# eRGiBi/DRL-DroneNavigation

Measured on AMD Instinct MI355X. Metric: env_steps_per_sec, higher is better.
Workload: dtype f64

## Files before the change

drl-dronenavigation_amd/csrc/dn_kernels.hip:

```cpp
#include "dn_internal.h"
#include "dn_action_sat.h"

#ifndef DN_TU
#define DN_TU 1
#endif

#include <float.h>
#include <type_traits>

#define DN_DEV __device__ __forceinline__

namespace {

template <typename R> struct K {
    static constexpr R M = R(0.027);
    static constexpr R IXX = R(1.4e-5), IYY = R(1.4e-5), IZZ = R(2.17e-5);
    static constexpr R G = R(9.8);
    static constexpr R DT = R(1.0 / 240.0);
    static constexpr R ARM = R(0.028);
    static constexpr R LIN_DAMP = R(0.04), ANG_DAMP = R(0.04);
    static constexpr R MAX_COORD_VEL = R(100.0);
    static constexpr R PI = R(3.14159265358979323846);
    static constexpr R COLL_R = R(0.06), COLL_H = R(0.025);
    static constexpr R INV_M = R(1.0 / 0.027);
// ... 543 lines not shown
    s = FM<R>::fma(s, h2, R(-1.0 / 6.0));
    sinc = FM<R>::fma(s, h2, R(1.0));
    R k = R(1.0 / 479001600.0);
    k = FM<R>::fma(k, h2, R(-1.0 / 3628800.0));
    k = FM<R>::fma(k, h2, R(1.0 / 40320.0));
    k = FM<R>::fma(k, h2, R(-1.0 / 720.0));
    k = FM<R>::fma(k, h2, R(1.0 / 24.0));
    k = FM<R>::fma(k, h2, R(-0.5));
    c = FM<R>::fma(k, h2, R(1.0));
}

struct Meta {
    int steps, idx, just_found;
};
DN_DEV Meta unpack_meta(float f)
{
    unsigned u = __float_as_uint(f);
    Meta m;
    m.steps = (int)(u & 0xFFFFFFu);
    m.idx = (int)((u >> 24) & 0x7Fu);
    m.just_found = (int)(u >> 31);
    return m;
}
DN_DEV float pack_meta(int steps, int idx, int just_found)
{
    return __uint_as_float(((unsigned)steps & 0xFFFFFFu) | (((unsigned)idx & 0x7Fu) << 24) | ((unsigned)just_found << 31));
}

struct StepOut {
    float *obs;
    float *reward;
    uint8_t *done, *truncated;
    int32_t *found;
    float *terminal_obs;
    float *ep_return;
    int32_t *ep_length;
    unsigned long long *done_word;
};
DN_DEV StepOut block_out(const DnStepIO &io, long long tile_base, long long step_off, long long word_off)
{
    StepOut o;
    const long long e = step_off + tile_base;
    o.obs = io.obs + e * DN_OBS_DIM;
    o.reward = io.reward + e;
    o.done = io.done + e;
    o.truncated = io.truncated + e;
    o.found = io.found_targets + e;
    o.terminal_obs = io.terminal_obs ? io.terminal_obs + e * DN_OBS_DIM : nullptr;
    o.ep_return = io.ep_return ? io.ep_return + e : nullptr;
    o.ep_length = io.ep_length ? io.ep_length + e : nullptr;
    o.done_word = io.done_mask ? io.done_mask + word_off + tile_base / DN_BLOCK : nullptr;
    return o;
}

DN_DEV void pin(double &x) { asm volatile("" : "+v"(x)); }
DN_DEV void pin(float &x) { asm volatile("" : "+v"(x)); }
DN_DEV void pin(bool &x) { int t = x; asm volatile("" : "+v"(t)); x = t != 0; }

DN_DEV void wave_lds_sync()
{
    __builtin_amdgcn_fence(__ATOMIC_RELEASE, "wavefront");
    __builtin_amdgcn_s_waitcnt(0xc07f);
    __builtin_amdgcn_wave_barrier();
    __builtin_amdgcn_fence(__ATOMIC_ACQUIRE, "wavefront");
}
DN_DEV void block_lds_barrier()
{
    __builtin_amdgcn_fence(__ATOMIC_RELEASE, "workgroup", "local");
    __builtin_amdgcn_s_barrier();
    __builtin_amdgcn_fence(__ATOMIC_ACQUIRE, "workgroup", "local");
}

DN_DEV void tile_park(float *s_tile, unsigned lane, const float o[DN_OBS_DIM])
{
    asm volatile("" ::: "memory");
#pragma unroll
    for (int k = 0; k < DN_OBS_DIM; ++k) s_tile[lane * DN_OBS_DIM + k] = o[k];
    asm volatile("" ::: "memory");
}
struct TileRegs {
    float4 r[4];
};
DN_DEV TileRegs tile_fetch(const float *s_tile, unsigned lane)
{
    asm volatile("" ::: "memory");
    const float4 *s4 = reinterpret_cast<const float4 *>(s_tile);
    TileRegs t;
#pragma unroll
    for (int r = 0; r < 3; ++r) t.r[r] = s4[r * 64 + lane];
    t.r[3] = s4[192 + (lane < (DN_BLOCK * DN_OBS_DIM / 4 - 192) ? lane : 0)];
    asm volatile("" ::: "memory");
    return t;
}
DN_DEV void tile_stream(const TileRegs &t, const float *s_tile, float *gtile, unsigned rows, unsigned lane)
{
    if (rows == DN_BLOCK) {
        float4 *g4 = reinterpret_cast<float4 *>(gtile);
#pragma unroll
        for (int r = 0; r < 3; ++r) g4[r * 64 + lane] = t.r[r];
        if (lane < (DN_BLOCK * DN_OBS_DIM / 4 - 192)) g4[192 + lane] = t.r[3];
    } else {
        const unsigned rem = rows * DN_OBS_DIM;
        for (unsigned e = lane; e < rem; e += DN_BLOCK) gtile[e] = s_tile[e];
    }
}
DN_DEV void store_obs_tile(float *s_tile, float *gtile, unsigned rows, unsigned lane, const float o[DN_OBS_DIM])
{
    tile_park(s_tile, lane, o);
    const TileRegs t = tile_fetch(s_tile, lane);
// ... 1176 lines not shown
        const double inv = rcp_f64(tot);
        const double delta = rn.returns - rn.mean;
        rn.mean = __builtin_fma(delta, inv, rn.mean);
        rn.var = __builtin_fma(delta * delta, inv, rn.var) * (rn.count * inv);
        rn.count = tot;
        const double s = rn.var + 1e-8;
        double y = __builtin_amdgcn_rsq(s);
        y = __builtin_fma(y, __builtin_fma(-(0.5 * s * y), y, 0.5), y);
        y = __builtin_fma(y, __builtin_fma(-(0.5 * s * y), y, 0.5), y);
        r = r * y;
        if (done) rn.returns = 0.0;
    }
    return r;
}

DN_DEV long long fixed6(double x)
{
    const double m = x * 1e6 + 6755399441055744.0;
    return __double_as_longlong(m) - 0x4338000000000000ll;
}

struct StatAcc {
    long long episodes = 0, truncated = 0, completed = 0, sum_len = 0, sum_found = 0, sum_ret_fix = 0;
};
DN_DEV void flush_stats(const DnParams &p, const StatAcc &a, unsigned long long steps_after, unsigned lane)
{
    if (lane == 0) {
        DnStatSlot sl = p.st.stats[blockIdx.x];
        sl.episodes += a.episodes; sl.truncated += a.truncated; sl.completed += a.completed;
        sl.sum_len += a.sum_len; sl.sum_found += a.sum_found; sl.sum_ret_fix += a.sum_ret_fix;
        sl.step_count = steps_after;
        p.st.stats[blockIdx.x] = sl;
    }
}
DN_DEV void flush_stats_preloaded(const DnParams &p, DnStatSlot sl, const StatAcc &a, unsigned long long steps_after, unsigned lane,
                                  const long long tile)
{
    if (lane == 0) {
        sl.episodes += a.episodes; sl.truncated += a.truncated; sl.completed += a.completed;
        sl.sum_len += a.sum_len; sl.sum_found += a.sum_found; sl.sum_ret_fix += a.sum_ret_fix;
        sl.step_count = steps_after;
        p.st.stats[tile] = sl;
    }
}

struct __attribute__((packed, aligned(4))) ObsQuad { float x, y, z, w; };
DN_DEV void store_obs_direct(float *row, const float o[DN_OBS_DIM])
{
    *reinterpret_cast<ObsQuad *>(row) = ObsQuad{o[0], o[1], o[2], o[3]};
    *reinterpret_cast<ObsQuad *>(row + 4) = ObsQuad{o[4], o[5], o[6], o[7]};
    *reinterpret_cast<ObsQuad *>(row + 8) = ObsQuad{o[8], o[9], o[10], o[11]};
    row[12] = o[12];
}
DN_DEV float ret_lo(const float hi, const int lenword)
{
    const int eb = (__float_as_int(hi) >> 23) & 0xFF;
    return (float)(lenword >> 24) * __int_as_float((eb > 31 ? eb - 31 : 0) << 23);
}
DN_DEV int ret_lo_byte(const double ep_ret, const float hi)
{
    const int eb = (__float_as_int(hi) >> 23) & 0xFF;
    const bool ok = eb > 31 && eb < 255;
    const float inv = __int_as_float((ok ? 285 - eb : 127) << 23);
    const double q = __builtin_rint((ep_ret - (double)hi) * (double)inv);
    const int k = (int)fmin(fmax(q, -128.0), 127.0);
    return ok ? (k & 0xFF) : 0;
}
template <typename R, bool REW, bool FOUND_BIT = false, bool BANK = false>
DN_DEV void report_scalars(const DnParams &p, const DnConsts<R> &c, const StepOut &out, const Flight<R> &fl, const Verdict<R> &v,
                           const R r_normal, const float r_found32, const unsigned li, const unsigned lane, const bool active,
                           float4 &G4, float4 &G5, StatAcc &acc, RewNorm &rn, const bool found_mail = false, const int W_lane = 0,
                           unsigned long long *track_count = nullptr, const int track_e = 0)
{
    const bool coll1 = v.coll1 != 0, terminated = v.terminated != 0, truncated = fl.truncated != 0;
    const bool found_now = !coll1 && (FOUND_BIT ? found_mail : (R)fl.d_e <= c.threshold);
    const bool is_done = found_now && fl.idx_e + 1 == (BANK ? W_lane : p.num_waypoints);
    const int found = fl.idx_e + (found_now ? 1 : 0);
    const bool done = terminated || truncated;
    R reward;
    if (coll1) reward = R(-10.0);
    else if (found_now) reward = (R)(r_found32 / 25.0f);
    else reward = r_normal * K<R>::INV_25;
    if (REW) reward = (R)reward_wrappers(p, rn, (double)reward, done);
    const int lenword = __float_as_int(G5.w);
    const int eplen_e = lenword & 0xFFFFFF;
    R ep_ret = ((R)G4.w + (R)ret_lo(G4.w, lenword)) + reward;
    int ep_len = eplen_e + 1;
    float4 S4 = G4, S5 = G5;
    if (!terminated) {
        S4 = make_float4(fl.vex, fl.vey, fl.vez, 0.0f);
        S5 = make_float4(fl.aex, fl.aey, fl.aez, 0.0f);
    }
    const unsigned long long done_ballot = __ballot(done && active);
    if (done_ballot != 0ull) {
        const long long fix = fixed6((double)ep_ret);
        if (done) {
            if (active) {
                if (out.ep_return) out.ep_return[li] = (float)ep_ret;
                if (out.ep_length) out.ep_length[li] = ep_len;
            }
            S4 = S5 = make_float4(0.0f, 0.0f, 0.0f, 0.0f);
            ep_ret = R(0.0); ep_len = 0;
        }
        const long long n_trunc = __popcll(__ballot(done && active && truncated && !terminated));
        const long long n_compl = __popcll(__ballot(done && active && is_done));
        long long s_len = 0, s_fd = 0, s_ret = 0;
        const int fix_lo = (int)(unsigned)(fix & 0xFFFFFFFFll), fix_hi = (int)(fix >> 32);
        for (unsigned long long m = done_ballot; m != 0ull; m &= m - 1ull) {
            const int l = __builtin_ctzll(m);
            s_len += (long long)__builtin_amdgcn_readlane(eplen_e, l) + 1;
            s_fd += (long long)__builtin_amdgcn_readlane(found, l);
            const unsigned lo = (unsigned)__builtin_amdgcn_readlane(fix_lo, l);
            const int hi = __builtin_amdgcn_readlane(fix_hi, l);
            s_ret += (long long)(((unsigned long long)(unsigned)hi << 32) | lo);
        }
        acc.episodes += __popcll(done_ballot); acc.truncated += n_trunc; acc.completed += n_compl;
        acc.sum_len += s_len; acc.sum_found += s_fd; acc.sum_ret_fix += s_ret;
        if constexpr (BANK) if (track_count) {
            for (unsigned long long left = done_ballot; left != 0ull;) {
                const int t = __builtin_amdgcn_readlane(track_e, __builtin_ctzll(left));
                const bool mine = done && active && track_e == t;
                const unsigned long long same = __ballot(mine);
                const unsigned long long c_compl = __popcll(__ballot(mine && is_done)), c_trunc = __popcll(__ballot(mine && truncated && !terminated));
                unsigned long long t_len = 0, t_fd = 0;
                for (unsigned long long m = same; m != 0ull; m &= m - 1ull) {
                    const int l = __builtin_ctzll(m);
                    t_len += (unsigned long long)(__builtin_amdgcn_readlane(eplen_e, l) + 1);
                    t_fd += (unsigned long long)__builtin_amdgcn_readlane(found, l);
                }
                if (lane == 0) {
                    unsigned long long *cnt = track_count + 5 * t;
                    track_count_add(cnt + 0, (unsigned long long)__popcll(same));
                    if (c_compl) track_count_add(cnt + 1, c_compl);
                    if (c_trunc) track_count_add(cnt + 2, c_trunc);
                    track_count_add(cnt + 3, t_fd);
                    track_count_add(cnt + 4, t_len);
                }
                left &= ~same;
            }
        }
    }
    S4.w = (float)ep_ret; S5.w = __int_as_float(ep_len | (ret_lo_byte((double)ep_ret, S4.w) << 24));
    G4 = S4; G5 = S5;
    if (active) {
        out.reward[li] = (float)reward;
        out.done[li] = (uint8_t)done;
        out.truncated[li] = (uint8_t)(truncated && !terminated);
        out.found[li] = found;
    }
    if (out.done_word && lane == 0) *out.done_word = done_ballot;
}
template <typename R, bool NORM, bool NOISE, int TILE, bool SPAWN = false, int M = DN_M_NONE>
DN_DEV void report_obs(const DnParams &p, const DnConsts<R> &c, float *s_tile, const StepOut &out, const bool truncated,
                       const Verdict<R> &v, float *o, const unsigned long long gid, const unsigned long long step_count,
                       const unsigned li, const unsigned lane, const unsigned rows, const bool active, Rms &rms, SensCtx *sx = nullptr,
                       const PrivCtx *px = nullptr, const GoalCtx<R> *gx = nullptr)
{
    constexpr bool SENS = M >= DN_M_SENS, PRIV = M >= DN_M_PRIV, GOAL = M >= DN_M_GOAL;
    const bool done = v.terminated != 0 || truncated;
    const unsigned long long done_mask = __ballot(done && active);
    if (done_mask != 0ull) {
        const bool across = NOISE && TILE == 2 && s_tile != nullptr && p.obs_noise_sigma > 0.0f;
        float zr[DN_OBS_DIM];
        if (across) draw_obs_noise_across(p, gid - li, step_count, 5u, done_mask, done && active, lane, s_tile, zr);
        if (done) {
            if (active && out.terminal_obs) {
#pragma unroll
                for (int k = 0; k < DN_OBS_DIM; ++k) out.terminal_obs[li * DN_OBS_DIM + k] = o[k];
            }
            reset_obs<R>(p, c, v.d_obs, o);
            if (SPAWN && p.random_spawn) {
                double q[3];
                spawn_point(p, gid, step_count, q);
#pragma unroll
                for (int k = 0; k < 3; ++k) o[k] = (float)((R)(float)q[k] * c.inv_dim[k]);
            }
            if constexpr (PRIV) {
                if ((px->pv->groups & DN_PRIV_OBS) && active) priv_store_obs(px->row, o);
            }
            if (across) add_obs_noise_drawn(p, zr, o);
            else if (NOISE && p.obs_noise_sigma > 0.0f) add_obs_noise(p, gid, step_count, 5u, o);
            if constexpr (SENS) {
                if (sx->sn->lat_on || sx->sn->bias_on)
                    sens_restart(*sx->sn, sx->n, sx->i, sx->active, p.seed, gid, step_count, sens_slot(*sx->sn, step_count), sx->d, o);
            }
            if constexpr (GOAL) {
                if (active && gx->row) goal_store<R>(*gx->g, gx->rW, c, gx->tab + gx->roff, gx->row, o, 0);
            }
            if (NORM) normalize_obs(rms, o);
        }
    }
    if (TILE == 2) { if (active) store_obs_direct(out.obs + li * DN_OBS_DIM, o); }
    else if (TILE == 1) tile_park(s_tile, lane, o);
    else store_obs_tile(s_tile, out.obs, rows, lane, o);
}
template <typename R, bool NORM, bool NOISE, bool REW, int TILE = 0, bool SPAWN = false, int M = DN_M_NONE>
DN_DEV void report_phase(const DnParams &p, const DnConsts<R> &c, float *s_tile, const StepOut &out, const Flight<R> &fl,
                         const Verdict<R> &v, Observed<R> &ob, const unsigned long long gid, const unsigned long long step_count,
                         const unsigned li, const unsigned lane, const unsigned rows, const bool active,
                         float4 &G4, float4 &G5, StatAcc &acc, Rms &rms, RewNorm &rn, SensCtx *sx = nullptr, const PrivCtx *px = nullptr,
                         const GoalCtx<R> *gx = nullptr, unsigned long long *track_count = nullptr, const int track_e = 0)
{
    if constexpr (M >= DN_M_GOAL) report_scalars<R, REW, false, true>(p, c, out, fl, v, ob.r_normal, ob.r_found32, li, lane, active, G4, G5, acc, rn, false, gx->W,
                                                                      track_count, track_e);
    else report_scalars<R, REW>(p, c, out, fl, v, ob.r_normal, ob.r_found32, li, lane, active, G4, G5, acc, rn);
    report_obs<R, NORM, NOISE, TILE, SPAWN, M>(p, c, s_tile, out, fl.truncated != 0, v, ob.o, gid, step_count, li, lane, rows, active,
                                                              rms, sx, px, gx);
}

struct BlockState {
    float4 *g0, *g1, *g2, *g3, *g4, *g5, *g6, *g7;
};
DN_DEV BlockState block_state(const DnState &st, long long tile_base)
{
    BlockState b;
    b.g0 = st.g0 + tile_base; b.g1 = st.g1 + tile_base; b.g2 = st.g2 + tile_base; b.g3 = st.g3 + tile_base;
    b.g4 = st.g4 + tile_base; b.g5 = st.g5 + tile_base; b.g6 = st.g6 + tile_base;
    b.g7 = st.g7 + tile_base;
    return b;
}

// ... 489 lines not shown
            if (XOPT && p.drag) G7 = (v.terminated || fl.truncated) ? make_float4(0.0f, 0.0f, 0.0f, 0.0f) : rpm_now;
            attitude_phase<R>(fl);
            post_mail<R>(mail[t & 1], lane, fl, v);
            block_lds_barrier();
            A = A_next;
        }
        if (active) { b.g0[li] = G0; b.g1[li] = G1; b.g2[li] = G2; b.g3[li] = G3; }
        if (XOPT && p.drag && active) b.g7[li] = G7;
    }
}

template <typename R> struct MailQ {
    R f64[8][DN_BLOCK];
    float4 f32[4][DN_BLOCK];
};
template <typename R> DN_DEV void post_mailq(MailQ<R> &m, unsigned lane, const Flight<R> &f, const Verdict<R> &v)
{
    const R x[8] = {f.px, f.py, f.pz, f.qx, f.qy, f.qz, f.qw, v.d_obs};
#pragma unroll
    for (int k = 0; k < 8; ++k) m.f64[k][lane] = x[k];
    const int fb = f.idx_e | (f.just_found_e << 8) | (f.truncated << 9), vb = v.coll1 | (v.terminated << 1);
    m.f32[0][lane] = make_float4(f.vx, f.vy, f.vz, f.wx);
    m.f32[1][lane] = make_float4(f.wy, f.wz, f.vex, f.vey);
    m.f32[2][lane] = make_float4(f.vez, f.aex, f.aey, f.aez);
    m.f32[3][lane] = make_float4(f.d_e, f.dprev_e, __int_as_float(fb), __int_as_float(vb));
}
template <typename R> DN_DEV void take_mailq(const MailQ<R> &m, unsigned lane, Flight<R> &f, Verdict<R> &v)
{
    R x[8];
#pragma unroll
    for (int k = 0; k < 8; ++k) x[k] = m.f64[k][lane];
    f.px = x[0]; f.py = x[1]; f.pz = x[2]; f.qx = x[3]; f.qy = x[4]; f.qz = x[5]; f.qw = x[6];
    v.d_obs = x[7];
    const float4 a = m.f32[0][lane], b = m.f32[1][lane], c = m.f32[2][lane], d = m.f32[3][lane];
    f.vx = a.x; f.vy = a.y; f.vz = a.z; f.wx = a.w; f.wy = b.x; f.wz = b.y; f.vex = b.z; f.vey = b.w;
    f.vez = c.x; f.aex = c.y; f.aey = c.z; f.aez = c.w; f.d_e = d.x; f.dprev_e = d.y;
    const int bits = __float_as_int(d.z), vb = __float_as_int(d.w);
    f.idx_e = bits & 0xFF; f.just_found_e = (bits >> 8) & 1; f.truncated = (bits >> 9) & 1;
    v.coll1 = vb & 1; v.terminated = (vb >> 1) & 1;
}
template <typename R> struct MailA {
    R f64[2][DN_BLOCK];
    float4 f32[4][DN_BLOCK];
};
template <typename R> DN_DEV void post_maila(MailA<R> &m, unsigned lane, const Flight<R> &f, const Verdict<R> &v, const Observed<R> &ob)
{
    m.f64[0][lane] = ob.r_normal; m.f64[1][lane] = v.d_obs;
    const int bits = f.idx_e | (f.truncated << 9) | (v.coll1 << 10) | (v.terminated << 11);
    m.f32[0][lane] = make_float4(ob.o[0], ob.o[1], ob.o[2], ob.o[3]);
    m.f32[1][lane] = make_float4(ob.o[4], ob.o[5], ob.o[6], ob.o[7]);
    m.f32[2][lane] = make_float4(ob.o[8], ob.o[9], ob.o[10], ob.o[11]);
    m.f32[3][lane] = make_float4(ob.o[12], ob.r_found32, f.d_e, __int_as_float(bits));
}
template <typename R> DN_DEV void take_maila(const MailA<R> &m, unsigned lane, Flight<R> &f, Verdict<R> &v, Observed<R> &ob, int *flag_word = nullptr)
{
    ob.r_normal = m.f64[0][lane]; v.d_obs = m.f64[1][lane];
    const float4 a = m.f32[0][lane], b = m.f32[1][lane], c = m.f32[2][lane], d = m.f32[3][lane];
    ob.o[0] = a.x; ob.o[1] = a.y; ob.o[2] = a.z; ob.o[3] = a.w; ob.o[4] = b.x; ob.o[5] = b.y; ob.o[6] = b.z; ob.o[7] = b.w;
    ob.o[8] = c.x; ob.o[9] = c.y; ob.o[10] = c.z; ob.o[11] = c.w; ob.o[12] = d.x;
    ob.r_found32 = d.y; f.d_e = d.z;
    const int bits = __float_as_int(d.w);
    f.idx_e = bits & 0xFF; f.truncated = (bits >> 9) & 1; v.coll1 = (bits >> 10) & 1; v.terminated = (bits >> 11) & 1;
    f.vex = f.vey = f.vez = f.aex = f.aey = f.aez = 0.0f;
    if (flag_word) *flag_word = bits;
}
constexpr int DN_MAILA_FOUND_SHIFT = 12;
template <typename R> DN_DEV void post_maila_found(MailA<R> &m, unsigned lane, const FlightW<R> &f, const Verdict<R> &v, const Observed<R> &ob,
                                                   const bool found)
{
    m.f64[0][lane] = ob.r_normal; m.f64[1][lane] = v.d_obs;
    const int bits = f.idx_e | (f.truncated << 9) | (v.coll1 << 10) | (v.terminated << 11) | ((int)found << DN_MAILA_FOUND_SHIFT);
    m.f32[0][lane] = make_float4(ob.o[0], ob.o[1], ob.o[2], ob.o[3]);
    m.f32[1][lane] = make_float4(ob.o[4], ob.o[5], ob.o[6], ob.o[7]);
    m.f32[2][lane] = make_float4(ob.o[8], ob.o[9], ob.o[10], ob.o[11]);
    m.f32[3][lane] = make_float4(ob.o[12], ob.r_found32, 0.0f, __int_as_float(bits));
}

template <bool XOPT> struct ThrustMailX { double v[9][DN_BLOCK]; };
template <> struct ThrustMailX<false> { double v[1][1]; };
DN_DEV void post_thrust_x(ThrustMailX<true> &m, unsigned lane, const ThrustX &t, const Extras &x)
{
#pragma unroll
    for (int j = 0; j < 4; ++j) { m.v[j][lane] = t.f[j]; m.v[5 + j][lane] = x.rpm[j]; }
    m.v[4][lane] = t.zt;
}
DN_DEV void take_thrust_x(const ThrustMailX<true> &m, unsigned lane, ThrustX &t, Extras &x)
{
#pragma unroll
    for (int j = 0; j < 4; ++j) { t.f[j] = m.v[j][lane]; x.rpm[j] = m.v[5 + j][lane]; }
    t.zt = m.v[4][lane];
}
DN_DEV void post_thrust_x(ThrustMailX<false> &, unsigned, const ThrustX &, const Extras &) {}
DN_DEV void take_thrust_x(const ThrustMailX<false> &, unsigned, ThrustX &, Extras &) {}
template <typename R, bool XOPT> struct ThrustMailP : ThrustMail<R> {};
template <typename R> struct ThrustMailP<R, true> { R v[1][1]; };
template <typename R> DN_DEV void post_thrust(ThrustMailP<R, true> &, unsigned, const Thrust &) {}
template <typename R> DN_DEV Resultant<R> take_thrust(const ThrustMailP<R, true> &, unsigned) { return Resultant<R>(); }

template <typename R, bool NORM, bool NOISE, bool XOPT>
__global__ __launch_bounds__(3 * DN_BLOCK, NORM ? 2 : 3) void dn_step_many_3w_kernel(const DnParams p, const DnStepIO io0, const int k_steps)
{
    __shared__ ThrustMailX<XOPT> tmx[2];
    __shared__ R s_tab[DN_MAX_WAYPOINTS * DN_T_STRIDE];
    __shared__ __attribute__((aligned(16))) float s_tile[DN_BLOCK * DN_OBS_DIM];
    __shared__ MailQ<R> mailq[2];
    __shared__ MailA<R> maila[2];
    __shared__ __attribute__((aligned(16))) ThrustMailP<R, XOPT> tmail[2];
    const unsigned lane = threadIdx.x & (DN_BLOCK - 1);
    const int wv = __builtin_amdgcn_readfirstlane(threadIdx.x >> 6);
    const int role = wv == 0 ? 0 : (wv == 1 ? 2 : 1);
    const long long tile_base = (long long)blockIdx.x * DN_BLOCK;
    const long long left = p.n - tile_base;
    const unsigned rows = left < DN_BLOCK ? (unsigned)left : DN_BLOCK;
    const bool active = lane < rows;
    const unsigned li = active ? lane : rows - 1;
// ... 120 lines not shown
            reinterpret_cast<float *>(b.g4 + li)[3] = G4.w;
            reinterpret_cast<float *>(b.g5 + li)[3] = G5.w;
            }
    }
}

template <typename R> struct MailL {
    R f64[4][DN_BLOCK];
    R wide[8][DN_BLOCK];
    int flags[DN_BLOCK];
};
template <typename R> struct MailG {
    R col[3][DN_BLOCK];
    R fw[3][DN_BLOCK];
    float4 eul[DN_BLOCK];
    float4 w[DN_BLOCK];
    R we[3][DN_BLOCK];
};

#ifdef DN_MW_STAMP
__device__ long long g_mw_stamp[8][48][2];
#define MW_MARK(k) do { if (lane == 0 && blockIdx.x == DN_MW_STAMP && t >= 8 && t < 56) \
        g_mw_stamp[role][t - 8][k] = (long long)__builtin_readcyclecounter(); } while (0)
#else
#define MW_MARK(k) do { } while (0)
#endif
#define MW_BARRIER() do { MW_MARK(0); block_lds_barrier(); MW_MARK(1); } while (0)
#ifdef DN_ROLE_MARK
#define MW_ROLE_MARK(name) asm volatile("; DN_ROLE_LOOP " name)
#else
#define MW_ROLE_MARK(name) do { } while (0)
#endif
#ifdef DN_MW_STAMP
__device__ long long g_mw_edge[16][8];
#define MW_EDGE(k) do { if (lane == 0 && (blockIdx.x == DN_MW_STAMP || blockIdx.x == DN_MW_STAMP + 256)) { const int r_ = role + (blockIdx.x == DN_MW_STAMP ? 0 : 8); \
        g_mw_edge[r_][k] = (long long)__builtin_readcyclecounter(); \
        if ((k) == 0) { g_mw_edge[r_][4] = (long long)wall_clock64(); g_mw_edge[r_][6] = (long long)__builtin_amdgcn_s_getreg(63492); } \
        if ((k) == 3) g_mw_edge[r_][5] = (long long)wall_clock64(); } } while (0)
#else
#define MW_EDGE(k) do { } while (0)
#endif

template <typename R, bool NORM, bool NOISE, int NW>
DN_DEV void step_many_4w_body(const DnParams &p, const DnStepIO &io0, const int k_steps)
{
    static_assert(NW == 4 || (NW == 5 && NORM), "the fifth wave is the normaliser's");
    __shared__ R s_tab[DN_MAX_WAYPOINTS * DN_T_STRIDE];
    __shared__ MailL<R> maill[2];
    __shared__ __attribute__((aligned(16))) MailG<R> mailg[2];
    __shared__ MailA<R> maila[2];
    __shared__ __attribute__((aligned(16))) ThrustMail<R> tmail[2];
    const unsigned lane = threadIdx.x & (DN_BLOCK - 1);
    constexpr bool THRUST_ON_Q = !NOISE || NORM;
    const int wv0 = __builtin_amdgcn_readfirstlane(threadIdx.x >> 6);
    const int second_tile = (int)((blockIdx.x / (unsigned)p.num_cus) & 1u);
    const int wv = (!NORM && second_tile) ? (wv0 ^ 2) : wv0;
#ifndef DN_5W_ORDER_A
#define DN_5W_ORDER_A "LQANX"
#define DN_5W_ORDER_B "ANLQX"
#endif
    int role;
    if (NW == 5) {
        constexpr char oa[6] = DN_5W_ORDER_A, ob[6] = DN_5W_ORDER_B;
        const char ch = second_tile ? ob[wv0] : oa[wv0];
        role = ch == 'L' ? 0 : ch == 'A' ? 1 : ch == 'Q' ? 2 : ch == 'X' ? 3 : 4;
    } else
        role = NORM ? (wv == 0 ? 0 : (wv == 1 ? 3 : (wv == 2 ? 1 : 2)))
                    : (wv == 0 ? 0 : (wv == 1 ? 1 : (wv == 2 ? 3 : 2)));
    const long long tile_base = (long long)blockIdx.x * DN_BLOCK;
    const long long left = p.n - tile_base;
    const unsigned rows = left < DN_BLOCK ? (unsigned)left : DN_BLOCK;
    const bool active = lane < rows;
    const unsigned li = active ? lane : rows - 1;
    __builtin_assume(li < DN_BLOCK);
    const long long i = tile_base + li;
    const unsigned long long gid = (unsigned long long)(p.env_id_offset + i);
    const BlockState b = block_state(p.st, tile_base);
    const DnConsts<R> &c = consts<R>(p);
    const long long n = p.n, words = (p.n + 63) / 64;
    const unsigned long long sc0 = p.st.stats[blockIdx.x].step_count;
    MW_EDGE(0);
    stage_table<R>(p, s_tab);
#ifndef DN_5W_PRIO
#define DN_5W_PRIO "22311"
#endif
    {
        constexpr char pr[6] = DN_5W_PRIO;
        switch (pr[role] - '0') {
        case 1: __builtin_amdgcn_s_setprio(1); break;
        case 2: __builtin_amdgcn_s_setprio(2); break;
        case 3: __builtin_amdgcn_s_setprio(3); break;
        default: break;
        }
    }
    if (role == 0) {
        float4 G0 = b.g0[li], G2 = b.g2[li], G3 = b.g3[li];
        AttCol<R> col = attitude_column<R>(b.g1[li]);
        block_lds_barrier(); MW_EDGE(1);
        const R wp0[3] = {s_tab[DN_T_WP], s_tab[DN_T_WP + 1], s_tab[DN_T_WP + 2]};
        bool done_prev = false;
        Vec3R<R> W2 = {(R)G2.x, (R)G2.y, (R)G2.z};
#pragma clang loop unroll(disable)
        for (int t = 0; t <= k_steps; ++t) {
            MW_ROLE_MARK("L");
            if (t < k_steps) {
                if (t > 0) {
                    const MailG<R> &mp = mailg[(t - 1) & 1];
                    const R c0 = mp.col[0][lane], c1 = mp.col[1][lane], c2 = mp.col[2][lane];
                    col.r02 = done_prev ? R(0.0) : c0; col.r12 = done_prev ? R(0.0) : c1; col.r22 = done_prev ? R(1.0) : c2;
                }
                const GateRow<R> row_e = load_gate_row<R>(s_tab, unpack_meta(G3.w).idx);
                const R fz = tmail[t & 1].v[0][lane];
                const Lin<R> lin = physics_linear_col<R>(G0, W2, col, fz, R(0.0), R(0.0), R(0.0), false);
                Flight<R> fl;
                flight_entry<R>(fl, G0, G2, G3, p.max_steps);
                fl.px = lin.px; fl.py = lin.py; fl.pz = lin.pz;
                fl.vx = (float)lin.vx; fl.vy = (float)lin.vy; fl.vz = (float)lin.vz;
                const Vec3R<R> Wn = {(R)fl.vx, (R)fl.vy, (R)fl.vz};
                fl.qx = fl.qy = fl.qz = R(0.0); fl.qw = R(1.0);
                fl.wx = fl.wy = fl.wz = 0.0f;
                RulesMid<R> m;
                const Verdict<R> v = rules_verdict<R>(p, c, s_tab, row_e, fl, G3, m);
                MailL<R> &ml = maill[t & 1];
                ml.f64[0][lane] = fl.px; ml.f64[1][lane] = fl.py; ml.f64[2][lane] = fl.pz; ml.f64[3][lane] = v.d_obs;
                ml.wide[0][lane] = Wn.x; ml.wide[1][lane] = Wn.y; ml.wide[2][lane] = Wn.z;
                ml.wide[3][lane] = W2.x; ml.wide[4][lane] = W2.y; ml.wide[5][lane] = W2.z;
                ml.wide[6][lane] = (R)fl.d_e; ml.wide[7][lane] = (R)fl.dprev_e;
                ml.flags[lane] = fl.idx_e | (fl.just_found_e << 8) | (fl.truncated << 9) | (v.coll1 << 10) | (v.terminated << 11);
                float4 S0, S1, S2, S3;
                rules_commit<R>(c, wp0, fl, m, G0, G3, b.g6, li, active, S0, S1, S2, S3);
                G0 = S0; G2 = S2; G3.w = S3.w;
                done_prev = v.terminated != 0 || fl.truncated != 0;
                W2 = Wn;
                if (__ballot(done_prev) != 0ull) {
                    if (done_prev) W2.x = W2.y = W2.z = R(0.0);
                }
            }
            MW_BARRIER();
        }
        MW_EDGE(2);
        if (active) {
            b.g0[li] = G0; b.g2[li] = G2;
            reinterpret_cast<float *>(b.g3 + li)[3] = G3.w;
        }
    } else if (role == 1) {
        float4 G1 = b.g1[li], G3 = b.g3[li];
        QuatTerms<R> qt = quat_terms<R>((R)G1.x, (R)G1.y, (R)G1.z, (R)G1.w);
        block_lds_barrier(); MW_EDGE(1);
#pragma clang loop unroll(disable)
        for (int t = 0; t <= k_steps; ++t) {
            MW_ROLE_MARK("A");
            if (t > 0) {
                const int fb = maill[(t - 1) & 1].flags[lane];
                const bool fin = (((fb >> 9) | (fb >> 11)) & 1) != 0;
                if (__ballot(fin) != 0ull) {
                    if (fin) { G1 = make_float4(0.0f, 0.0f, 0.0f, 1.0f); G3.x = G3.y = G3.z = 0.0f; qt = quat_terms_identity<R>(); }
                }
            }
            if (t < k_steps) {
                MailG<R> &mg = mailg[t & 1];
                mg.we[0][lane] = (R)G3.x; mg.we[1][lane] = (R)G3.y; mg.we[2][lane] = (R)G3.z;
                const R tx = tmail[t & 1].v[1][lane], ty = tmail[t & 1].v[2][lane], zt = tmail[t & 1].v[3][lane];
                const Ang<R> ang = physics_angular_post<R>(physics_angular_pre_terms<R>(G1, G3, qt), tx, ty, zt);
                Flight<R> fl;
                fl.qx = ang.qx; fl.qy = ang.qy; fl.qz = ang.qz; fl.qw = ang.qw;
                attitude_phase<R>(fl);
                const float4 qn = make_float4((float)ang.qx, (float)ang.qy, (float)ang.qz, (float)ang.qw);
                const float4 wn = make_float4((float)ang.wx, (float)ang.wy, (float)ang.wz, 0.0f);
                qt = quat_terms<R>((R)qn.x, (R)qn.y, (R)qn.z, (R)qn.w);
                const AttCol<R> cn = attitude_column_terms<R>(qn, qt);
                mg.col[0][lane] = cn.r02; mg.col[1][lane] = cn.r12; mg.col[2][lane] = cn.r22;
                mg.fw[0][lane] = fl.fwx; mg.fw[1][lane] = fl.fwy; mg.fw[2][lane] = fl.fwz;
                mg.eul[lane] = make_float4(fl.roll_num32, fl.roll_den32, fl.pitch32, fl.yaw32);
                mg.w[lane] = wn;
                G1 = qn; G3.x = wn.x; G3.y = wn.y; G3.z = wn.z;
            }
            MW_BARRIER();
        }
        MW_EDGE(2);
        if (active) {
            b.g1[li] = G1;
            float *g3 = reinterpret_cast<float *>(b.g3 + li);
            g3[0] = G3.x; g3[1] = G3.y; g3[2] = G3.z;
        }
    } else if (role == 2) {
        Vec3R<R> P4, P5;
        {
            const float4 g4 = b.g4[li], g5 = b.g5[li];
            P4.x = (R)g4.x; P4.y = (R)g4.y; P4.z = (R)g4.z; P5.x = (R)g5.x; P5.y = (R)g5.y; P5.z = (R)g5.z;
        }
        const float4 *act = reinterpret_cast<const float4 *>(io0.actions) + tile_base;
        float4 A = make_float4(0.0f, 0.0f, 0.0f, 0.0f);
        if (THRUST_ON_Q) {
            A = act[li];
            const float4 A1 = (act + (long long)(k_steps > 1 ? 1 : 0) * n)[li];
            post_thrust<R>(tmail[0], lane, thrust_phase<NOISE>(p, gid, sc0, A));
            A = A1;
        }
        block_lds_barrier(); MW_EDGE(1);
#pragma clang loop unroll(disable)
        for (int t = 0; t <= k_steps; ++t) {
            MW_ROLE_MARK("Q");
            if (THRUST_ON_Q && t + 1 < k_steps) {
                const float4 A_next = (act + (long long)(t + 2 < k_steps ? t + 2 : t + 1) * n)[li];
                post_thrust<R>(tmail[(t + 1) & 1], lane, thrust_phase<NOISE>(p, gid, sc0 + (unsigned long long)(t + 1), A));
                A = A_next;
            }
            if (t > 0) {
                const int u = t - 1;
                const MailL<R> &ml = maill[u & 1];
                const MailG<R> &mg = mailg[u & 1];
                FlightW<R> fl;
                Verdict<R> v;
                fl.px = ml.f64[0][lane]; fl.py = ml.f64[1][lane]; fl.pz = ml.f64[2][lane]; v.d_obs = ml.f64[3][lane];
                fl.vx = ml.wide[0][lane]; fl.vy = ml.wide[1][lane]; fl.vz = ml.wide[2][lane];
                fl.vex = ml.wide[3][lane]; fl.vey = ml.wide[4][lane]; fl.vez = ml.wide[5][lane];
                fl.d_e = ml.wide[6][lane]; fl.dprev_e = ml.wide[7][lane];
                const int fb = ml.flags[lane];
                fl.idx_e = fb & 0xFF; fl.just_found_e = (fb >> 8) & 1; fl.truncated = (fb >> 9) & 1;
                v.coll1 = (fb >> 10) & 1; v.terminated = (fb >> 11) & 1;
                const float4 e = mg.eul[lane], wn = mg.w[lane];
                fl.qx = fl.qy = fl.qz = R(0.0); fl.qw = R(1.0);
                fl.fwx = mg.fw[0][lane]; fl.fwy = mg.fw[1][lane]; fl.fwz = mg.fw[2][lane];
                fl.roll_num32 = e.x; fl.roll_den32 = e.y; fl.pitch32 = e.z; fl.yaw32 = e.w;
                fl.wx = wn.x; fl.wy = wn.y; fl.wz = wn.z;
                fl.aex = mg.we[0][lane]; fl.aey = mg.we[1][lane]; fl.aez = mg.we[2][lane];
                Observed<R> ob;
                observe_columns_lin<R>(p, c, fl, ob.o);
                observe_columns_att<R>(fl, ob.o);
                const RewardPre<R> pre = reward_entry<R>(p, c, fl, P4, P5);
                reward_pose<R>(p, s_tab, fl, pre, ob.r_normal, ob.r_found32);
                if (NOISE && p.obs_noise_sigma > 0.0f) add_obs_noise(p, gid, sc0 + (unsigned long long)u, 1u, ob.o);
                post_maila_found<R>(maila[u & 1], lane, fl, v, ob, pre.found_now);
                {
                    const bool fin = v.terminated != 0 || fl.truncated != 0;
                    P4.x = fin ? R(0.0) : fl.vex; P4.y = fin ? R(0.0) : fl.vey; P4.z = fin ? R(0.0) : fl.vez;
                    P5.x = fin ? R(0.0) : fl.aex; P5.y = fin ? R(0.0) : fl.aey; P5.z = fin ? R(0.0) : fl.aez;
                }
            }
            MW_BARRIER();
        }
        MW_EDGE(2);
        if (active) {
            float *g4 = reinterpret_cast<float *>(b.g4 + li), *g5 = reinterpret_cast<float *>(b.g5 + li);
            g4[0] = (float)P4.x; g4[1] = (float)P4.y; g4[2] = (float)P4.z; g5[0] = (float)P5.x; g5[1] = (float)P5.y; g5[2] = (float)P5.z;
        }
    } else if (role == 4) {
        Rms rms;
        load_rms(p, i, rms);
        block_lds_barrier(); MW_EDGE(1);
#pragma clang loop unroll(disable)
        for (int t = 0; t <= k_steps + 1; ++t) {
            MW_ROLE_MARK("N");
            if (t > 1) {
                const int u = t - 2;
                Flight<R> fl;
                Verdict<R> v;
                Observed<R> ob;
                take_maila<R>(maila[u & 1], lane, fl, v, ob);
                normalize_obs(rms, ob.o);
                const StepOut out = block_out(io0, tile_base, (long long)u * n, (long long)u * words);
                report_obs<R, NORM, NOISE, 2>(p, c, nullptr, out, fl.truncated != 0, v, ob.o, gid, sc0 + (unsigned long long)u, li, lane, rows, active, rms);
            }
            if (t <= k_steps) MW_BARRIER();
        }
        MW_EDGE(2);
        if (active) store_rms(p, i, rms);
    } else {
        float4 G4 = b.g4[li], G5 = b.g5[li];
        StatAcc acc;
        Rms rms;
        if (NORM && NW == 4) load_rms_walk(p, tile_base, li, rms);
        RewNorm rn = {0.0, 0.0, 1.0, 1e-4};
        const float4 *act = reinterpret_cast<const float4 *>(io0.actions) + tile_base;
        float4 A = make_float4(0.0f, 0.0f, 0.0f, 0.0f);
        if (!THRUST_ON_Q) {
            A = act[li];
            const float4 A1 = (act + (long long)(k_steps > 1 ? 1 : 0) * n)[li];
            post_thrust<R>(tmail[0], lane, thrust_phase<NOISE>(p, gid, sc0, A));
            A = A1;
        }
        block_lds_barrier(); MW_EDGE(1);
#pragma clang loop unroll(disable)
        for (int t = 0; t <= k_steps + 1; ++t) {
            MW_ROLE_MARK("X");
            if (!THRUST_ON_Q && t + 1 < k_steps) {
                const float4 A_next = (act + (long long)(t + 2 < k_steps ? t + 2 : t + 1) * n)[li];
                post_thrust<R>(tmail[(t + 1) & 1], lane, thrust_phase<NOISE>(p, gid, sc0 + (unsigned long long)(t + 1), A));
                A = A_next;
            }
            if (t > 1) {
                const int u = t - 2;
                const unsigned long long sc = sc0 + (unsigned long long)u;
                Flight<R> fl;
                Verdict<R> v;
                Observed<R> ob;
                int fb;
                take_maila<R>(maila[u & 1], lane, fl, v, ob, &fb);
                const bool found_mail = ((fb >> DN_MAILA_FOUND_SHIFT) & 1) != 0;
                const StepOut out = block_out(io0, tile_base, (long long)u * n, (long long)u * words);
                if (NW != 5 && NORM) normalize_obs(rms, ob.o);
                report_scalars<R, false, true>(p, c, out, fl, v, ob.r_normal, ob.r_found32, li, lane, active, G4, G5, acc, rn, found_mail);
                if (NW != 5)
                    report_obs<R, NORM, NOISE, 2>(p, c, nullptr, out, fl.truncated != 0, v, ob.o, gid, sc, li, lane, rows, active, rms);
            }
            if (t <= k_steps) MW_BARRIER();
        }
        MW_EDGE(2);
        flush_stats(p, acc, sc0 + (unsigned long long)k_steps, lane);
        if (NORM && NW == 4 && active) store_rms_walk(p, tile_base, li, rms);
        if (active) {
            reinterpret_cast<float *>(b.g4 + li)[3] = G4.w;
            reinterpret_cast<float *>(b.g5 + li)[3] = G5.w;
        }
    }
    MW_EDGE(3);
}

template <typename R, bool NORM, bool NOISE>
__global__ __launch_bounds__(4 * DN_BLOCK, 2) void dn_step_many_4w_kernel(const DnParams p, const DnStepIO io0, const int k_steps)
{
    step_many_4w_body<R, NORM, NOISE, 4>(p, io0, k_steps);
}
template <typename R, bool NOISE>
#ifndef DN_5W_WAVES_PER_EU
#define DN_5W_WAVES_PER_EU 4
#endif
__global__ __launch_bounds__(5 * DN_BLOCK) __attribute__((amdgpu_waves_per_eu(DN_5W_WAVES_PER_EU, DN_5W_WAVES_PER_EU))) void dn_step_many_5w_kernel(const DnParams p, const DnStepIO io0, const int k_steps)
{
    step_many_4w_body<R, true, NOISE, 5>(p, io0, k_steps);
}

template <typename R> struct RMailL {
    R f64[5][DN_BLOCK];
    float4 f32[DN_BLOCK];
};
template <typename R> struct RMailA {
    R q[4][DN_BLOCK];
    R col[3][DN_BLOCK];
    float4 w[DN_BLOCK];
    float4 we[DN_BLOCK];
};
template <typename R> struct RMailE {
    float4 oa[DN_BLOCK];
    float4 ob[DN_BLOCK];
};
template <typename R> struct RMailC {
    R r[4][DN_BLOCK];
    float4 oa[DN_BLOCK];
    float4 ob[DN_BLOCK];
};
struct __attribute__((packed, aligned(4))) ObsTri { float x, y, z; };

template <typename R>
DN_DEV bool found_from_d2(const DnConsts<R> &c, const R d2)
{
    bool found = d2 < c.thr2;
// ... 1185 lines not shown
```

Measured before the change: 25.95 billion.

## Walk output pointers incrementally and use nontemporal stores in multi-wave step kernel

Adds strided pointer walkers that keep per-step output and action addresses in scalar registers and advance them each step, replacing the 64-bit address recomputation done every step. Output stores can be made nontemporal (on by default). In the 5-wave lean path, the per-lane selects that zero state on episode reset are put behind a wave ballot, and the mail flags are re-unpacked from pinned values. The aim is fewer VALU and SGPR address instructions in the role loops, at the cost of more template complexity and possible cache effects from nontemporal stores.

New measurement: 26.23 billion, median of 6. 1.01x the previous value.

```diff
diff --git a/drl-dronenavigation_amd/csrc/dn_kernels.hip b/drl-dronenavigation_amd/csrc/dn_kernels.hip
--- a/drl-dronenavigation_amd/csrc/dn_kernels.hip
+++ b/drl-dronenavigation_amd/csrc/dn_kernels.hip
@@ -619,9 +619,84 @@
     o.done_word = io.done_mask ? io.done_mask + word_off + tile_base / DN_BLOCK : nullptr;
     return o;
 }
+#ifndef DN_STEP_OUT_NT
+#define DN_STEP_OUT_NT 1
+#endif
+template <typename T> struct WalkRef {
+    T *p;
+    DN_DEV void operator=(const T v) const
+    {
+        if (DN_STEP_OUT_NT) __builtin_nontemporal_store(v, p);
+        else *p = v;
+    }
+};
+template <typename T> struct WalkRow {
+    T *p;
+    DN_DEV operator T *() const { return p; }
+};
+template <typename T> struct WalkPtr {
+    typedef __attribute__((address_space(1))) char GlobalByte;
+    typedef __attribute__((address_space(1))) T GlobalT;
+    unsigned long long at, stride;
+    DN_DEV void set(T *p, const long long per_step) { at = (unsigned long long)p; stride = p ? (unsigned long long)per_step * sizeof(T) : 0ull; }
+    DN_DEV void advance() { at += stride; asm volatile("" : "+s"(at)); }
+    DN_DEV T *lane(const unsigned k) const
+    {
+        unsigned b = k * (unsigned)sizeof(T);
+        asm volatile("" : "+v"(b));
+        return (T *)(GlobalT *)((GlobalByte *)at + b);
+    }
+    DN_DEV explicit operator bool() const { return at != 0ull; }
+    DN_DEV operator T *() const { return lane(0u); }
+    DN_DEV WalkRef<T> operator[](const unsigned k) const { return WalkRef<T>{lane(k)}; }
+    DN_DEV WalkRow<T> operator+(const unsigned k) const { return WalkRow<T>{lane(k)}; }
+    DN_DEV WalkRef<T> operator*() const { return WalkRef<T>{lane(0u)}; }
+};
+template <bool ROWS, bool SCALARS>
+struct StepOutWalk {
+    WalkPtr<float> obs, reward;
+    WalkPtr<uint8_t> done, truncated;
+    WalkPtr<int32_t> found;
+    WalkPtr<float> terminal_obs, ep_return;
+    WalkPtr<int32_t> ep_length;
+    WalkPtr<unsigned long long> done_word;
+    DN_DEV StepOutWalk(const DnStepIO &io, const long long tile_base, const long long n, const long long words)
+    {
+        const StepOut o = block_out(io, tile_base, 0, 0);
+        obs.set(o.obs, n * DN_OBS_DIM); terminal_obs.set(o.terminal_obs, n * DN_OBS_DIM);
+        reward.set(o.reward, n); done.set(o.done, n); truncated.set(o.truncated, n); found.set(o.found, n);
+        ep_return.set(o.ep_return, n); ep_length.set(o.ep_length, n); done_word.set(o.done_word, words);
+    }
+    DN_DEV void advance()
+    {
+        if (ROWS) { obs.advance(); terminal_obs.advance(); }
+        if (SCALARS) {
+            reward.advance(); done.advance(); truncated.advance(); found.advance();
+            ep_return.advance(); ep_length.advance(); done_word.advance();
+        }
+    }
+};
+template <int K0, int K1, bool ROWS, bool SCALARS>
+DN_DEV void store_terminal_cols(const StepOutWalk<ROWS, SCALARS> &out, const float *o)
+{
+    float *row = out.terminal_obs + __builtin_amdgcn_mbcnt_hi(~0u, __builtin_amdgcn_mbcnt_lo(~0u, 0u)) * DN_OBS_DIM;
+#pragma unroll
+    for (int k = K0; k < K1; ++k) row[k] = o[k];
+}
+struct ActionWalk {
+    WalkPtr<const float4> row;
+    DN_DEV ActionWalk(const float4 *act, const long long n, const int k_steps) { row.set(act + (long long)(k_steps > 2 ? 2 : (k_steps > 1 ? 1 : 0)) * n, n); }
+    DN_DEV float4 take(const unsigned li, const int t, const int k_steps)
+    {
+        const float4 a = *row.lane(li);
+        if (t + 3 < k_steps) row.advance();
+        return a;
+    }
+};
 
 DN_DEV void pin(double &x) { asm volatile("" : "+v"(x)); }
 DN_DEV void pin(float &x) { asm volatile("" : "+v"(x)); }
+DN_DEV void pin(int &x) { asm volatile("" : "+v"(x)); }
 DN_DEV void pin(bool &x) { int t = x; asm volatile("" : "+v"(t)); x = t != 0; }
 
 DN_DEV void wave_lds_sync()
@@ -1904,6 +1979,18 @@
     *reinterpret_cast<ObsQuad *>(row + 8) = ObsQuad{o[8], o[9], o[10], o[11]};
     row[12] = o[12];
 }
+DN_DEV void store_obs_direct(const WalkRow<float> row, const float o[DN_OBS_DIM])
+{
+    if (DN_STEP_OUT_NT) {
+        typedef float Quad __attribute__((ext_vector_type(4)));
+        typedef Quad QuadA4 __attribute__((aligned(4)));
+        __builtin_nontemporal_store(Quad{o[0], o[1], o[2], o[3]}, reinterpret_cast<QuadA4 *>(row.p));
+        __builtin_nontemporal_store(Quad{o[4], o[5], o[6], o[7]}, reinterpret_cast<QuadA4 *>(row.p + 4));
+        __builtin_nontemporal_store(Quad{o[8], o[9], o[10], o[11]}, reinterpret_cast<QuadA4 *>(row.p + 8));
+        __builtin_nontemporal_store(o[12], row.p + 12);
+    } else
+        store_obs_direct(row.p, o);
+}
 DN_DEV float ret_lo(const float hi, const int lenword)
 {
     const int eb = (__float_as_int(hi) >> 23) & 0xFF;
@@ -1918,8 +2005,8 @@
     const int k = (int)fmin(fmax(q, -128.0), 127.0);
     return ok ? (k & 0xFF) : 0;
 }
-template <typename R, bool REW, bool FOUND_BIT = false, bool BANK = false>
-DN_DEV void report_scalars(const DnParams &p, const DnConsts<R> &c, const StepOut &out, const Flight<R> &fl, const Verdict<R> &v,
+template <typename R, bool REW, bool FOUND_BIT = false, bool BANK = false, typename OUT = StepOut>
+DN_DEV void report_scalars(const DnParams &p, const DnConsts<R> &c, const OUT &out, const Flight<R> &fl, const Verdict<R> &v,
                            const R r_normal, const float r_found32, const unsigned li, const unsigned lane, const bool active,
                            float4 &G4, float4 &G5, StatAcc &acc, RewNorm &rn, const bool found_mail = false, const int W_lane = 0,
                            unsigned long long *track_count = nullptr, const int track_e = 0)
@@ -2002,8 +2089,8 @@
     }
     if (out.done_word && lane == 0) *out.done_word = done_ballot;
 }
-template <typename R, bool NORM, bool NOISE, int TILE, bool SPAWN = false, int M = DN_M_NONE>
-DN_DEV void report_obs(const DnParams &p, const DnConsts<R> &c, float *s_tile, const StepOut &out, const bool truncated,
+template <typename R, bool NORM, bool NOISE, int TILE, bool SPAWN = false, int M = DN_M_NONE, typename OUT = StepOut>
+DN_DEV void report_obs(const DnParams &p, const DnConsts<R> &c, float *s_tile, const OUT &out, const bool truncated,
                        const Verdict<R> &v, float *o, const unsigned long long gid, const unsigned long long step_count,
                        const unsigned li, const unsigned lane, const unsigned rows, const bool active, Rms &rms, SensCtx *sx = nullptr,
                        const PrivCtx *px = nullptr, const GoalCtx<R> *gx = nullptr)
@@ -2017,8 +2104,11 @@
         if (across) draw_obs_noise_across(p, gid - li, step_count, 5u, done_mask, done && active, lane, s_tile, zr);
         if (done) {
             if (active && out.terminal_obs) {
-#pragma unroll
-                for (int k = 0; k < DN_OBS_DIM; ++k) out.terminal_obs[li * DN_OBS_DIM + k] = o[k];
+                if constexpr (std::is_same_v<OUT, StepOut>) {
+#pragma unroll
+                    for (int k = 0; k < DN_OBS_DIM; ++k) out.terminal_obs[li * DN_OBS_DIM + k] = o[k];
+                } else
+                    store_terminal_cols<0, DN_OBS_DIM>(out, o);
             }
             reset_obs<R>(p, c, v.d_obs, o);
             if (SPAWN && p.random_spawn) {
@@ -2614,6 +2704,10 @@
     m.f32[2][lane] = make_float4(ob.o[8], ob.o[9], ob.o[10], ob.o[11]);
     m.f32[3][lane] = make_float4(ob.o[12], ob.r_found32, f.d_e, __int_as_float(bits));
 }
+template <typename R> DN_DEV void unpack_maila_flags(const int bits, Flight<R> &f, Verdict<R> &v)
+{
+    f.idx_e = bits & 0xFF; f.truncated = (bits >> 9) & 1; v.coll1 = (bits >> 10) & 1; v.terminated = (bits >> 11) & 1;
+}
 template <typename R> DN_DEV void take_maila(const MailA<R> &m, unsigned lane, Flight<R> &f, Verdict<R> &v, Observed<R> &ob, int *flag_word = nullptr)
 {
     ob.r_normal = m.f64[0][lane]; v.d_obs = m.f64[1][lane];
@@ -2622,7 +2716,7 @@
     ob.o[8] = c.x; ob.o[9] = c.y; ob.o[10] = c.z; ob.o[11] = c.w; ob.o[12] = d.x;
     ob.r_found32 = d.y; f.d_e = d.z;
     const int bits = __float_as_int(d.w);
-    f.idx_e = bits & 0xFF; f.truncated = (bits >> 9) & 1; v.coll1 = (bits >> 10) & 1; v.terminated = (bits >> 11) & 1;
+    unpack_maila_flags<R>(bits, f, v);
     f.vex = f.vey = f.vez = f.aex = f.aey = f.aez = 0.0f;
     if (flag_word) *flag_word = bits;
 }
@@ -2849,6 +2943,10 @@
     __shared__ __attribute__((aligned(16))) ThrustMail<R> tmail[2];
     const unsigned lane = threadIdx.x & (DN_BLOCK - 1);
     constexpr bool THRUST_ON_Q = !NOISE || NORM;
+    constexpr bool LEAN = NW == 5;
+    struct NoWalk { DN_DEV NoWalk(...) {} };
+    typedef std::conditional_t<LEAN, ActionWalk, NoWalk> ActionWalkIf;
+    typedef std::conditional_t<LEAN, StepOutWalk<false, true>, NoWalk> StepOutWalkIf;
     const int wv0 = __builtin_amdgcn_readfirstlane(threadIdx.x >> 6);
     const int second_tile = (int)((blockIdx.x / (unsigned)p.num_cus) & 1u);
     const int wv = (!NORM && second_tile) ? (wv0 ^ 2) : wv0;
@@ -2896,6 +2994,7 @@
         block_lds_barrier(); MW_EDGE(1);
         const R wp0[3] = {s_tab[DN_T_WP], s_tab[DN_T_WP + 1], s_tab[DN_T_WP + 2]};
         bool done_prev = false;
+        unsigned long long reset_prev = 0ull;
         Vec3R<R> W2 = {(R)G2.x, (R)G2.y, (R)G2.z};
 #pragma clang loop unroll(disable)
         for (int t = 0; t <= k_steps; ++t) {
@@ -2904,7 +3003,14 @@
                 if (t > 0) {
                     const MailG<R> &mp = mailg[(t - 1) & 1];
                     const R c0 = mp.col[0][lane], c1 = mp.col[1][lane], c2 = mp.col[2][lane];
-                    col.r02 = done_prev ? R(0.0) : c0; col.r12 = done_prev ? R(0.0) : c1; col.r22 = done_prev ? R(1.0) : c2;
+                    if constexpr (LEAN) {
+                        col.r02 = c0; col.r12 = c1; col.r22 = c2;
+                        if (reset_prev != 0ull) {
+                            if (done_prev) { col.r02 = R(0.0); col.r12 = R(0.0); col.r22 = R(1.0); }
+                        }
+                    } else {
+                        col.r02 = done_prev ? R(0.0) : c0; col.r12 = done_prev ? R(0.0) : c1; col.r22 = done_prev ? R(1.0) : c2;
+                    }
                 }
                 const GateRow<R> row_e = load_gate_row<R>(s_tab, unpack_meta(G3.w).idx);
                 const R fz = tmail[t & 1].v[0][lane];
@@ -2929,7 +3035,8 @@
                 G0 = S0; G2 = S2; G3.w = S3.w;
                 done_prev = v.terminated != 0 || fl.truncated != 0;
                 W2 = Wn;
-                if (__ballot(done_prev) != 0ull) {
+                reset_prev = __ballot(done_prev);
+                if (reset_prev != 0ull) {
                     if (done_prev) W2.x = W2.y = W2.z = R(0.0);
                 }
             }
@@ -2994,12 +3101,15 @@
             post_thrust<R>(tmail[0], lane, thrust_phase<NOISE>(p, gid, sc0, A));
             A = A1;
         }
+        ActionWalkIf act_walk(act, n, k_steps);
         block_lds_barrier(); MW_EDGE(1);
 #pragma clang loop unroll(disable)
         for (int t = 0; t <= k_steps; ++t) {
             MW_ROLE_MARK("Q");
             if (THRUST_ON_Q && t + 1 < k_steps) {
-                const float4 A_next = (act + (long long)(t + 2 < k_steps ? t + 2 : t + 1) * n)[li];
+                float4 A_next;
+                if constexpr (LEAN) A_next = act_walk.take(li, t, k_steps);
+                else A_next = (act + (long long)(t + 2 < k_steps ? t + 2 : t + 1) * n)[li];
                 post_thrust<R>(tmail[(t + 1) & 1], lane, thrust_phase<NOISE>(p, gid, sc0 + (unsigned long long)(t + 1), A));
                 A = A_next;
             }
@@ -3031,8 +3141,15 @@
                 post_maila_found<R>(maila[u & 1], lane, fl, v, ob, pre.found_now);
                 {
                     const bool fin = v.terminated != 0 || fl.truncated != 0;
-                    P4.x = fin ? R(0.0) : fl.vex; P4.y = fin ? R(0.0) : fl.vey; P4.z = fin ? R(0.0) : fl.vez;
-                    P5.x = fin ? R(0.0) : fl.aex; P5.y = fin ? R(0.0) : fl.aey; P5.z = fin ? R(0.0) : fl.aez;
+                    if constexpr (LEAN) {
+                        P4.x = fl.vex; P4.y = fl.vey; P4.z = fl.vez; P5.x = fl.aex; P5.y = fl.aey; P5.z = fl.aez;
+                        if (__ballot(fin) != 0ull) {
+                            if (fin) { P4.x = P4.y = P4.z = R(0.0); P5.x = P5.y = P5.z = R(0.0); }
+                        }
+                    } else {
+                        P4.x = fin ? R(0.0) : fl.vex; P4.y = fin ? R(0.0) : fl.vey; P4.z = fin ? R(0.0) : fl.vez;
+                        P5.x = fin ? R(0.0) : fl.aex; P5.y = fin ? R(0.0) : fl.aey; P5.z = fin ? R(0.0) : fl.aez;
+                    }
                 }
             }
             MW_BARRIER();
@@ -3045,6 +3162,7 @@
     } else if (role == 4) {
         Rms rms;
         load_rms(p, i, rms);
+        StepOutWalk<true, false> walk(io0, tile_base, n, words);
         block_lds_barrier(); MW_EDGE(1);
 #pragma clang loop unroll(disable)
         for (int t = 0; t <= k_steps + 1; ++t) {
@@ -3056,8 +3174,8 @@
                 Observed<R> ob;
                 take_maila<R>(maila[u & 1], lane, fl, v, ob);
                 normalize_obs(rms, ob.o);
-                const StepOut out = block_out(io0, tile_base, (long long)u * n, (long long)u * words);
-                report_obs<R, NORM, NOISE, 2>(p, c, nullptr, out, fl.truncated != 0, v, ob.o, gid, sc0 + (unsigned long long)u, li, lane, rows, active, rms);
+                report_obs<R, NORM, NOISE, 2>(p, c, nullptr, walk, fl.truncated != 0, v, ob.o, gid, sc0 + (unsigned long long)u, li, lane, rows, active, rms);
+                walk.advance();
             }
             if (t <= k_steps) MW_BARRIER();
         }
@@ -3077,6 +3195,7 @@
             post_thrust<R>(tmail[0], lane, thrust_phase<NOISE>(p, gid, sc0, A));
             A = A1;
         }
+        StepOutWalkIf walk(io0, tile_base, n, words);
         block_lds_barrier(); MW_EDGE(1);
 #pragma clang loop unroll(disable)
         for (int t = 0; t <= k_steps + 1; ++t) {
@@ -3094,12 +3213,20 @@
                 Observed<R> ob;
                 int fb;
                 take_maila<R>(maila[u & 1], lane, fl, v, ob, &fb);
+                if (LEAN) {
+                    pin(fb); pin(ob.r_normal); pin(ob.r_found32);
+                    unpack_maila_flags<R>(fb, fl, v);
+                }
                 const bool found_mail = ((fb >> DN_MAILA_FOUND_SHIFT) & 1) != 0;
-                const StepOut out = block_out(io0, tile_base, (long long)u * n, (long long)u * words);
-                if (NW != 5 && NORM) normalize_obs(rms, ob.o);
-                report_scalars<R, false, true>(p, c, out, fl, v, ob.r_normal, ob.r_found32, li, lane, active, G4, G5, acc, rn, found_mail);
-                if (NW != 5)
+                if constexpr (LEAN) {
+                    report_scalars<R, false, true>(p, c, walk, fl, v, ob.r_normal, ob.r_found32, li, lane, active, G4, G5, acc, rn, found_mail);
+                    walk.advance();
+                } else {
+                    const StepOut out = block_out(io0, tile_base, (long long)u * n, (long long)u * words);
+                    if (NORM) normalize_obs(rms, ob.o);
+                    report_scalars<R, false, true>(p, c, out, fl, v, ob.r_normal, ob.r_found32, li, lane, active, G4, G5, acc, rn, found_mail);
                     report_obs<R, NORM, NOISE, 2>(p, c, nullptr, out, fl.truncated != 0, v, ob.o, gid, sc, li, lane, rows, active, rms);
+                }
             }
             if (t <= k_steps) MW_BARRIER();
         }
diff --git a/profiles/role_overhead.py b/profiles/role_overhead.py
--- /dev/null
+++ b/profiles/role_overhead.py
@@ -0,0 +1,54 @@
+#!/usr/bin/env python3
+import os
+import subprocess
+import sys
+import tempfile
+
+sys.path.insert(0, os.path.dirname(os.path.abspath(__file__)))
+import role_cvt
+
+COLUMNS = (
+    ("VALU", lambda op, arg: op.startswith("v_")),
+    ("cndmask", lambda op, arg: op.startswith("v_cndmask")),
+    ("v_mov", lambda op, arg: op.startswith("v_mov")),
+    ("addr64", lambda op, arg: op.startswith(("v_lshl_add_u64", "v_mad_u64_u32", "v_add_co", "v_addc_co"))),
+    ("s_mul", lambda op, arg: op.startswith("s_mul_")),
+    ("lgkm wait", lambda op, arg: op == "s_waitcnt" and "lgkmcnt" in arg),
+    ("LDS rd", lambda op, arg: op.startswith("ds_read")),
+    ("LDS wr", lambda op, arg: op.startswith("ds_write")),
+    ("glb ld", lambda op, arg: op.startswith("global_load")),
+    ("glb st", lambda op, arg: op.startswith("global_store")),
+)
+
+
+def table(loops):
+    print(f"{'role':4} " + " ".join(f"{name:>9}" for name, _ in COLUMNS))
+    tot = [0] * len(COLUMNS)
+    for role in "LAQNX":
+        row = [0] * len(COLUMNS)
+        for ins in loops[role]:
+            op, arg = (ins.split(None, 1) + [""])[:2]
+            for j, (_, hit) in enumerate(COLUMNS):
+                row[j] += bool(hit(op, arg))
+        tot = [a + b for a, b in zip(tot, row)]
+        print(f"{role:4} " + " ".join(f"{v:9d}" for v in row))
+    print(f"{'sum':4} " + " ".join(f"{v:9d}" for v in tot))
+
+
+def main(argv):
+    if "--asm" in argv:
+        table(role_cvt.role_loops(argv[argv.index("--asm") + 1]))
+        return
+    with tempfile.TemporaryDirectory() as t:
+        out = os.path.join(t, "mw.s")
+        r = subprocess.run(["hipcc"] + role_cvt.FLAGS + argv + [os.path.join(role_cvt.ROOT, "drl-dronenavigation_amd", "csrc", "dn_kernels_mw.hip"), "-o", out],
+                           stderr=subprocess.PIPE, text=True)
+        if r.returncode != 0:
+            sys.exit(r.stderr)
+        table(role_cvt.role_loops(out))
+        print("dn_step_many_5w_kernel<double, false>:")
+        role_cvt.resources(r.stderr)
+
+
+if __name__ == "__main__":
+    main(sys.argv[1:])
diff --git a/profiles/role_spills.py b/profiles/role_spills.py
--- /dev/null
+++ b/profiles/role_spills.py
@@ -0,0 +1,69 @@
+#!/usr/bin/env python3
+import os
+import re
+import subprocess
+import sys
+import tempfile
+
+sys.path.insert(0, os.path.dirname(os.path.abspath(__file__)))
+import role_cvt
+
+KERNEL = re.compile(r"^(_ZN12_GLOBAL__N_122dn_step_many_[45]w_kernelI\w+):")
+
+
+def kernels(path):
+    return [m.group(1) for m in (KERNEL.match(l) for l in open(path)) if m]
+
+
+def pretty(name):
+    m = re.search(r"many_(\dw)_kernelI([df])((?:Lb[01]E)+)", name)
+    flags = re.findall(r"Lb([01])E", m.group(3))
+    names = ("NORM", "NOISE") if m.group(1) == "4w" else ("NOISE",)
+    return f"{m.group(1)}<{'double' if m.group(2) == 'd' else 'float'}" + "".join(f", {n}={f}" for n, f in zip(names, flags)) + ">"
+
+
+def loops_of(path, kern):
+    text = open(path).read()
+    body = text[text.index("\n" + kern + ":"):]
+    body = body[:body.index("\n.Lfunc_end")]
+    roles = "".join(r for r in "LAQNX" if f"; DN_ROLE_LOOP {r}" in body)
+    saved = role_cvt.KERN
+    role_cvt.KERN = kern
+    try:
+        if roles == "LAQNX":
+            return role_cvt.role_loops(path)
+        with tempfile.NamedTemporaryFile("w", suffix=".s") as f:
+            f.write(body[1:] + "\n.LBB999999_0:\n\t; DN_ROLE_LOOP N\n\ts_nop 0\n\ts_branch .LBB999999_0\n.Lfunc_end:\n")
+            f.flush()
+            loops = role_cvt.role_loops(f.name)
+        loops.pop("N")
+        return loops
+    finally:
+        role_cvt.KERN = saved
+
+
+def table(path):
+    print(f"{'kernel':34} {'role':4} {'all':>5} {'readlane':>9} {'writelane':>10} {'scratch':>8}")
+    for kern in kernels(path):
+        for role, ins in loops_of(path, kern).items():
+            rd = sum(bool(re.match(r"v_readlane_b32\s+s\d+,\s*v\d+,\s*\d+", x)) for x in ins)
+            wr = sum(x.startswith("v_writelane_b32") for x in ins)
+            sc = sum(x.startswith(("scratch_load", "scratch_store")) for x in ins)
+            print(f"{pretty(kern):34} {role:4} {len(ins):5d} {rd:9d} {wr:10d} {sc:8d}")
+
+
+def main(argv):
+    if "--asm" in argv:
+        table(argv[argv.index("--asm") + 1])
+        return
+    with tempfile.TemporaryDirectory() as t:
+        out = os.path.join(t, "mw.s")
+        r = subprocess.run(["hipcc"] + role_cvt.FLAGS + argv + [os.path.join(role_cvt.ROOT, "drl-dronenavigation_amd", "csrc", "dn_kernels_mw.hip"), "-o", out],
+                           stderr=subprocess.PIPE, text=True)
+        if r.returncode != 0:
+            sys.exit(r.stderr)
+        table(out)
+
+
+if __name__ == "__main__":
+    main(sys.argv[1:])
```
